# ThotDjehuty/polaroid

Hardware: AMD Instinct MI355X
Metric: Mrows/sec filter+groupby-agg on 1e9-row f64/i64; achieved HBM GB/s vs peak (higher is better)
Workload: dtype f64; 1 GPU; filter(close > 250).group_by(symbol).agg(open/high/low/close.sum()) 1e+09 rows per GPU, 100 groups (metric size; configs[1] = 1e8 rows); rows_per_gpu=1000000000, groups=100, global_batch=1000000000, columns=symbol:i64 open,high,low,close:f64, parallelism=single GPU

## Files before the change

### polaroid_amd/csrc/groupby.hip

```cpp
#include <hip/hip_runtime.h>

#include <algorithm>
#include <cmath>
#include <cstdio>
#include <cstdlib>
#include <cstring>
#include <mutex>
#include <numeric>
#include <string>
#include <tuple>
#include <vector>

#include "groupby_kernels.hpp"

namespace plgpu {

static int d2h_stage(int n, void* const* dst, const void* const* src, const size_t* bytes, hipStream_t s) {
    return plgpu_memcpy_d2h_many(n, dst, src, bytes, (void*)s);
}


#ifdef PLGPU_CHECKS
static std::vector<GbChecksTake>& gb_checks_takers() {
    static std::vector<GbChecksTake> v;
// ... 622 lines not shown
                }
                if ((x & 0x7fffffffffffffffull) != 0 && ex != 0x7FF && el < mn) mn = el;
            }
        }
    }
#pragma unroll
    for (int off = 32; off >= 1; off >>= 1) {
        const uint32_t o = __shfl_xor(mx, off, 64);
        mx = mx > o ? mx : o;
        const uint32_t q = __shfl_xor(mn, off, 64);
        mn = mn < q ? mn : q;
    }
    if ((threadIdx.x & 63) == 0) {
        red[0][threadIdx.x >> 6] = mx;
        red[1][threadIdx.x >> 6] = mn;
    }
    __syncthreads();
    if (threadIdx.x == 0) {
        for (int w = 1; w < kPlanThreads / 64; ++w) {
            mx = red[0][w] > mx ? red[0][w] : mx;
            mn = red[1][w] < mn ? red[1][w] : mn;
        }
        if (mx) atomicMax((unsigned long long*)&p.status[ST_MAXEX + a], (unsigned long long)mx);
        if (mn != 0x7FF) atomicMax((unsigned long long*)&p.status[ST_MINEX + a], (unsigned long long)(0x7FF - mn));
    }
}

static int32_t plan_bottom(uint64_t maxex) {
    int e = maxex == 0 ? 2046 : (int)maxex + kHeadroomBinades;
    if (e > 2046) e = 2046;
    return e - 1075 - (kSumWindowBits - 53);
}

__global__ void gb_init_table_kernel(uint64_t* gtab, int64_t words_per_field, int nfields, uint64_t min_init_mask) {
    for (int f = 0; f < nfields; ++f) {
        const uint64_t v = f == 0 ? kEmptyKey : (((min_init_mask >> f) & 1ull) ? ~0ull : 0ull);
        uint64_t* q = gtab + (int64_t)f * words_per_field;
        for (int64_t i = (int64_t)blockIdx.x * blockDim.x + threadIdx.x; i < words_per_field;
             i += (int64_t)gridDim.x * blockDim.x)
            q[i] = v;
    }
}


constexpr int kVarWords = 16;

__device__ __forceinline__ bool abs192(uint64_t& w0, uint64_t& w1, uint64_t& w2) {
    const bool neg = (int64_t)w2 < 0;
    if (neg) {
        w0 = ~w0; w1 = ~w1; w2 = ~w2;
        w0 += 1;
        const uint64_t c0 = w0 == 0;
        w1 += c0;
        w2 += (c0 && w1 == 0) ? 1 : 0;
    }
    return neg;
}

__device__ bool big_add_shifted(uint64_t (&acc)[kVarWords], const uint64_t* m, int k, int sh, bool negate) {
    int top = k - 1;
    while (top >= 0 && m[top] == 0) --top;
    if (top < 0) return true;
    const int bitlen = top * 64 + 64 - __clzll(m[top]);
    if (sh < 0 || bitlen + sh > kVarWords * 64 - 2) return false;
    const int ws = sh >> 6, bs = sh & 63;
    uint64_t carry = negate ? 1 : 0;
    for (int i = 0; i < kVarWords; ++i) {
// ... 786 lines not shown
            continue;
        }
        if (lp.n != 3 || lp.code[2].arg != PLGPU_F64) continue;
        int32_t op;
        switch (lp.code[2].op) {
        case D_ADD_F: op = DOP_ADD; break;
        case D_SUB_F: op = DOP_SUB; break;
        case D_MUL_F: op = DOP_MUL; break;
        case D_DIV_F: op = DOP_DIV; break;
        case D_DIV_FS: op = DOP_DIVS; break;
        default: continue;
        }
        const DevInstr &i0 = lp.code[0], &i1 = lp.code[1];
        auto f64col = [&](const DevInstr& i) { return i.op == D_COL && cols[i.arg].dtype == PLGPU_F64; };
        if (f64col(i0) && f64col(i1)) {
            di.kind = 2, di.ca = i0.arg, di.cb = i1.arg, di.dop = op;
        } else if (f64col(i0) && i1.op == D_LIT) {
            di.kind = 2, di.ca = i0.arg, di.dop = op | DOP_LIT, di.imm = i1.imm;
        } else if (i0.op == D_LIT && f64col(i1)) {
            di.kind = 2, di.ca = i1.arg, di.dop = op | DOP_LIT | DOP_SWAP, di.imm = i0.imm;
        }
    }
    return PLGPU_OK;
}

struct GbRun {
    Plan pl;
    DevProgram dp;
    int pred = 0;
    hipStream_t s = nullptr;
    DevBuf<uint64_t> status;
    int32_t* bottoms = nullptr;
    DevBuf<uint64_t> gtab;
    uint64_t st[ST_WORDS];
    int32_t hb[kMaxAcc];
    int gbits = 10;
    int attempts = 0;
    float ms = 0.f;
    int32_t key_dtype = PLGPU_I64;
    bool maintain = false;
    bool want_first = false;
    int world = 1;
    uint32_t wide = 0;
    int wide_exmin[kMaxAcc] = {0};
    int wide_exmax[kMaxAcc] = {0};
    DevBuf<int64_t> wide_digits[kMaxAcc];
    DevBuf<double> wide_sum[kMaxAcc];
    int64_t est_groups = -1;
    bool wide_round = true;
    std::string plan_ckey;
    bool kp_fallback = false;
    bool kp_bad = false;
    bool part = false;
    int pbits = 0;
    int part_lbits = 0;
    int part_blocks = 1;
    int part_levels = 0;
    int rbits = 0;
    bool compact_ok = false;
    bool compact_now = false;
    DevBuf<uint32_t> region_cnt;
    DevBuf<uint64_t> rtab;
    bool has_null_key = false;
    int64_t null_key = 0;
    DevBuf<uint64_t> pbuf;
    DevBuf<uint64_t> prange;
// ... 800 lines not shown
                                  160 * 1024);
        attr_set = true;
    }
    DevProgram none;
    std::memset(&none, 0, sizeof none);
    gb_kernel<0, true, true><<<(1 << R.pbits) * R.part_blocks, kGbThreads, lds, R.s>>>(q, none);
    return hipGetLastError();
}

static int gb_alloc_table(GbRun& R) {
    GbParams& p = R.pl.p;
    R.gtab.reset();
    R.rtab.reset();
    p.rtab = nullptr;
    p.rcap = 0;
    p.region_cnt = nullptr;
    p.gbits = R.gbits;
    p.rbits = R.rbits;
    if (R.compact_now) {
        p.rcap = int64_t(1) << (R.pbits + R.part_lbits);
        int rc = R.rtab.alloc((size_t)p.rcap * p.nfields * 8, R.s);
        if (rc) return rc;
        p.rtab = R.rtab;
        p.region_cnt = R.region_cnt;
        p.gbits = std::max(16, R.pbits + 2);
        p.rbits = 0;
    }
    p.gcap = int64_t(1) << p.gbits;
    const size_t wpf = (size_t)(p.gcap + 2);
    int rc = R.gtab.alloc(wpf * p.nfields * 8, R.s);
    if (rc) return rc;
    p.gtab = R.gtab;
    const int ig = (int)std::min<int64_t>((int64_t)(wpf + 255) / 256, 256 * 8);
    gb_init_table_kernel<<<ig, 256, 0, R.s>>>(R.gtab, (int64_t)wpf, p.nfields, p.min_init_mask);
    PLGPU_HIP(hipMemsetAsync(R.status, 0, 6 * 8, R.s));
    PLGPU_HIP(hipMemsetAsync(R.status + ST_MAXEX, 0, (ST_WORDS - ST_MAXEX) * 8, R.s));
    PLGPU_HIP(hipGetLastError());
    return PLGPU_OK;
}

static int gb_refit(GbRun& R, uint32_t flagged, int32_t* hint, bool* changed, uint32_t* wide) {
    GbParams& p = R.pl.p;
    *changed = false;
    *wide = 0;
    for (int a = 0; a < kMaxAcc; ++a) hint[a] = R.hb[a];
    if (!flagged) return PLGPU_OK;
    for (int a = 0; a < p.nacc; ++a)
        if ((flagged >> a) & 1u) gb_maxexp_kernel<<<std::max(1, num_cus() * 4), 256, 0, R.s>>>(p, a);
    PLGPU_HIP(hipGetLastError());
    if (int rs = d2h_status(R)) return rs;
    for (int a = 0; a < p.nacc; ++a) {
        if (!((flagged >> a) & 1u)) continue;
        const int tmax = std::max((int)R.st[ST_MAXEX + a], 1);
        const int tmin = std::max(0x7FF - (int)R.st[ST_MINEX + a], 1);
        if (tmax - tmin <= kSumWindowBits - 53) {
            hint[a] = tmax - 1075 - (kSumWindowBits - 53);
            *changed = *changed || hint[a] != R.hb[a];
        } else {
            *wide |= 1u << a;
            R.wide_exmin[a] = std::min(tmin, tmax);
            R.wide_exmax[a] = tmax;
        }
    }
    return PLGPU_OK;
}

static int gb_wide(GbRun& R, bool round = true) {
// ... 1743 lines not shown
```

### polaroid_amd/csrc/groupby_kernels.hpp

```cpp
#pragma once
#include <hip/hip_runtime.h>

#include <algorithm>
#include <cmath>
#include <cstdio>
#include <cstdlib>
#include <cstring>
#include <mutex>
#include <numeric>
#include <optional>
#include <string>
#include <tuple>
#include <vector>

#include "plgpu_internal.hpp"
#include "scan.hpp"
#include "tuplehash.hpp"

namespace plgpu {

constexpr int kGbThreads = 512;
constexpr int kMaxAcc = 6;
constexpr int kMaxFields = 48;
constexpr int kLdsProbe = 16;
constexpr int kGlobalProbe = 4096;
constexpr int kLimb2Margin = 4;
constexpr int slim_vwords(int nacc) { return (1 + 3 * nacc) | 1; }
constexpr int slim_words(int nacc) { return 1 + slim_vwords(nacc); }
constexpr int kMinTilesPerWg = 160;
constexpr int kGridRounds = 8;
constexpr int kHeadroomBinades = 8;
constexpr int64_t kMaxRowsPerWg = int64_t(1) << 22;
constexpr int kPlanSamples = 65536;
constexpr int kPlanSetSlots = 4096;
constexpr int kPlanSetWord = 32;

enum : int32_t { A_FSUM = 1, A_FSUMCAST = 2, A_ISUM = 4, A_CNT = 8, A_MIN = 16, A_MAX = 32, A_FLAGS = 64 };
enum : uint8_t { FOP_NONE = 0, FOP_ADD = 1, FOP_MIN = 2, FOP_MAX = 3, FOP_OR = 4, FOP_ADD192 = 5, FOP_SKIP = 6 };
enum : uint32_t { FL_NAN = 1, FL_PINF = 2, FL_NINF = 4 };
enum : int {
    ST_NEWKEYS = 0,
    ST_GLOBAL_ROWS = 1,
    ST_TABLE_FULL = 2,
    ST_SELECTED = 3,
    ST_SPECIAL = 4,
    ST_GROUPS_OUT = 5,
    ST_DISTINCT = 6,
    ST_SAMPLED = 7,
    ST_MAXEX = 8,
    ST_FXFLAGS = 16,
    ST_SHIFT_OVF = 14,
    ST_MINEX = 17,
    ST_RUNS = 23,
    ST_LOCAL = 24,
    ST_VAR_OUT = 25,
    ST_KPACK = 26,
    ST_WORDS = 27
};

enum : int32_t { DOP_NONE = 0, DOP_ADD = 1, DOP_SUB = 2, DOP_MUL = 3, DOP_DIV = 4, DOP_DIVS = 5, DOP_SQHI = 6,
                 DOP_SQLO = 7, DOP_OPMASK = 7, DOP_SWAP = 8, DOP_LIT = 16 };

struct AccSpec {
    DevCol c;
    int32_t flags;
// ... 39 lines not shown
    int32_t _pad2;
    int32_t nacc;
    int32_t nfields;
    AccSpec acc[kMaxAcc];
    uint64_t desc[kMaxAcc];
    int32_t bottom[kMaxAcc];
    uint8_t fop[kMaxFields];
    int32_t pred_acc;
    int32_t f_len;
    int32_t f_first;
    int32_t f_last;
    int32_t lbits;
    uint64_t min_init_mask;
    int32_t lcap;
    int32_t gbits;
    int64_t gcap;
    uint64_t* gtab;
    const int32_t* bottoms;
    uint64_t* status;
    const uint64_t* part_range;
    const uint32_t* part_rows;
    const uint8_t* part_nulls;
    int32_t part_blocks;
    int32_t tiles_per_wg;
    int32_t rbits;
    int32_t vwords;
    KeyPack kp;
    uint32_t* region_cnt;
    uint64_t* rtab;
    int64_t rcap;
    int32_t wave_report;
    int32_t has_null_key;
    int64_t null_key;
};

enum : uint32_t {
    CK_LDS_SLOT = 1,
    CK_GLOBAL_SLOT = 2,
    CK_FAST_SLOT = 4,
    CK_FIRST_ROW = 8,
    CK_MERGE_SLOT = 16,
    CK_REP_ROW = 32,
    CK_VERIFY_SLOT = 64,
    CK_PART_POS = 128,
    CK_KEY_ROW = 256,
    CK_PERM = 512,
    CK_FIELD = 1024,
    CK_REGION = 2048
};
#ifdef PLGPU_CHECKS
using GbChecksTake = uint32_t (*)();
void gb_checks_register(GbChecksTake f);
static __device__ unsigned int g_gb_checks;
static __device__ unsigned long long g_gb_sink;
static uint32_t gb_checks_take_local() {
    uint32_t v = 0, z = 0;
    (void)hipMemcpyFromSymbol(&v, HIP_SYMBOL(g_gb_checks), sizeof v);
    (void)hipMemcpyToSymbol(HIP_SYMBOL(g_gb_checks), &z, sizeof z);
    return v;
}
static const bool g_gb_checks_registered = (gb_checks_register(&gb_checks_take_local), true);
__device__ __forceinline__ bool gb_ok(bool c, uint32_t bit) {
    if (!c) atomicOr(&g_gb_checks, bit);
    return c;
}
__device__ __forceinline__ unsigned long long* gb_sink() { return &g_gb_sink; }
// ... 610 lines not shown
                if (s >= 0) {
                    apply_row<true, kMaxAcc>(p, lds, L, s, row, rv, vm[0], dd, bot, nacc, d);
                } else {
                    ++d.nglobal;
                    global_row<kMaxAcc>(p, key[0], s != kGlobalNull, row, rv, vm[0], dd, bot, nacc, d);
                }
            }
            slot[0] = slot[1]; slot[1] = slot[2]; slot[2] = slot[3];
            vm[0] = vm[1]; vm[1] = vm[2]; vm[2] = vm[3];
            key[0] = key[1]; key[1] = key[2]; key[2] = key[3];
#pragma unroll
            for (int a = 0; a < kMaxAcc; ++a) {
                v[a][0] = v[a][1];
                v[a][1] = v[a][2];
                v[a][2] = v[a][3];
            }
        }
    }
    flush_and_report<USE_LDS>(p, lds, L, d);
}

constexpr int kKpFast = 2;
template <int NACC, int ROWS, bool DERIV = false, int PACK = 0, bool NUL = false>
struct FastTile {
    uint64_t key[ROWS];
    uint64_t kr[PACK ? kKpFast : 1][ROWS];
    uint64_t v[NACC > 0 ? NACC : 1][ROWS];
    uint64_t w[DERIV && NACC > 0 ? NACC : 1][ROWS];
    uint64_t pv[ROWS];
    uint32_t nv[NUL ? (ROWS + 1) / 2 : 1];
    uint32_t nr[NUL ? (ROWS + 1) / 2 : 1][NUL ? (NACC > 0 ? NACC : 1) + 2 : 1];
};

__device__ __forceinline__ int64_t fast_row(int64_t t, int T, int rows, int j) {
    return t * (int64_t)T * rows + (int64_t)(j >> 1) * 2 * T + 2 * threadIdx.x + (j & 1);
}

typedef unsigned long long u64x2_t __attribute__((ext_vector_type(2)));

template <bool NT>
__device__ __forceinline__ u64x2_t ld16(const uint64_t* p) {
    if (NT) return __builtin_nontemporal_load(reinterpret_cast<const u64x2_t*>(p));
    return *reinterpret_cast<const u64x2_t*>(p);
}

template <int NACC, int PRED, int ROWS, bool DERIV, int PACK, bool NUL = false>
__device__ __forceinline__ void fast_load_tail(const GbParams& p, int64_t t,
                                               FastTile<NACC, ROWS, DERIV, PACK, NUL>& x) {
    const int T = blockDim.x;
    const uint64_t* kp = (const uint64_t*)p.key.values + p.key.offset;
#pragma unroll
    for (int j = 0; j < ROWS; ++j) {
        const int64_t r = fast_row(t, T, ROWS, j);
        const bool in = r < p.n;
        if (PACK == 2) {
            const int64_t* o = (const int64_t*)p.kp.c[0].values + p.kp.c[0].offset;
            x.kr[0][j] = in ? (uint64_t)o[r] : 0ull;
            x.kr[1][j] = in ? (uint64_t)o[r + 1] : 0ull;
        } else if (PACK == 1) {
#pragma unroll
            for (int i = 0; i < kKpFast; ++i) x.kr[i][j] = in && i < p.kp.n ? dev_load(p.kp.c[i], r) : 0ull;
        } else {
            x.key[j] = in && p.key.values ? kp[r] : 0ull;
        }
#pragma unroll
        for (int c = 0; c < NACC; ++c) {
            if (!DERIV || p.acc[c].v_from < 0)
                x.v[c][j] = in ? ((const uint64_t*)p.acc[c].c.values + p.acc[c].c.offset)[r] : 0ull;
            if (DERIV && p.acc[c].dop != DOP_NONE && !(p.acc[c].dop & DOP_LIT) && p.acc[c].w_from < 0)
                x.w[c][j] = in ? ((const uint64_t*)p.acc[c].c2.values + p.acc[c].c2.offset)[r] : 0ull;
        }
        if (PRED == 1 && p.pred_acc < 0) x.pv[j] = in ? ((const uint64_t*)p.pred_col.values + p.pred_col.offset)[r] : 0ull;
    }
}

typedef unsigned int u32x2_t __attribute__((ext_vector_type(2)));

template <int NACC, int PRED, int ROWS, bool NT, bool DERIV, int PACK, bool NUL = false>
__device__ __forceinline__ void fast_load(const GbParams& p, int64_t t, FastTile<NACC, ROWS, DERIV, PACK, NUL>& x,
                                          int64_t rbase = 0, int64_t rmax = -1) {
    const int T = blockDim.x;
    const uint64_t* kp = (const uint64_t*)p.key.values + p.key.offset;
#pragma unroll
    for (int q = 0; q < ROWS / 2; ++q) {
        int64_t r = rbase + fast_row(t, T, ROWS, 2 * q);
        if (rmax >= 0) r = r < rmax ? r : rmax;
        if (PACK == 2) {
            const int64_t* o = (const int64_t*)p.kp.c[0].values + p.kp.c[0].offset + r;
            const u64x2_t a = ld16<NT>((const uint64_t*)o);
            const uint64_t e = NT ? __builtin_nontemporal_load((const uint64_t*)o + 2) : ((const uint64_t*)o)[2];
            x.kr[0][2 * q] = a.x;
            x.kr[0][2 * q + 1] = a.y;
            x.kr[1][2 * q] = a.y;
            x.kr[1][2 * q + 1] = e;
        } else if (PACK == 1) {
#pragma unroll
            for (int i = 0; i < kKpFast; ++i) {
                if (i >= p.kp.n) {
                    x.kr[i][2 * q] = x.kr[i][2 * q + 1] = 0;
                    continue;
                }
                const DevCol& kc = p.kp.c[i];
                if (kc.dtype == PLGPU_I64) {
                    const u64x2_t a = ld16<NT>((const uint64_t*)kc.values + kc.offset + r);
                    x.kr[i][2 * q] = a.x;
                    x.kr[i][2 * q + 1] = a.y;
                } else {
                    const u32x2_t* ap = reinterpret_cast<const u32x2_t*>((const uint32_t*)kc.values + kc.offset + r);
                    const u32x2_t a = NT ? __builtin_nontemporal_load(ap) : *ap;
                    x.kr[i][2 * q] = a.x;
                    x.kr[i][2 * q + 1] = a.y;
                }
            }
        } else if (p.key.values) {
            const u64x2_t a = ld16<NT>(kp + r);
            x.key[2 * q] = a.x;
            x.key[2 * q + 1] = a.y;
        } else {
// ... 11 lines not shown
                const uint64_t* wp = (const uint64_t*)p.acc[c].c2.values + p.acc[c].c2.offset;
                const u64x2_t w = ld16<NT>(wp + r);
                x.w[c][2 * q] = w.x;
                x.w[c][2 * q + 1] = w.y;
            }
        }
        if (PRED == 1 && p.pred_acc < 0) {
            const uint64_t* pp = (const uint64_t*)p.pred_col.values + p.pred_col.offset;
            const u64x2_t b = ld16<NT>(pp + r);
            x.pv[2 * q] = b.x;
            x.pv[2 * q + 1] = b.y;
        }
    }
}

__device__ __forceinline__ uint64_t pair_bit(const DevCol& c, int64_t r) {
    return ((uint64_t)(uintptr_t)c.validity & 3u) * 8u + (uint64_t)(c.offset + r);
}

__device__ __forceinline__ uint32_t pair_word(const DevCol& c, int64_t r) {
    if (!c.validity) return ~0u;
    const uint32_t* w = (const uint32_t*)((uintptr_t)c.validity & ~(uintptr_t)3);
    return __builtin_nontemporal_load(w + (pair_bit(c, r) >> 5));
}

__device__ __forceinline__ uint32_t pair_word_wave(const DevCol& c, int64_t rw) {
    if (!c.validity) return ~0u;
    const int lane = threadIdx.x & 63;
    const uint64_t b = (uint64_t)(c.offset + rw) + 2u * (uint32_t)lane;
    return __builtin_nontemporal_load((const uint32_t*)c.validity + (b >> 5));
}

template <int NACC, int PRED, int ROWS, bool PART, bool DERIV, int PACK, bool NUL>
__device__ __forceinline__ void fast_nulls(const GbParams& p, int64_t t, FastTile<NACC, ROWS, DERIV, PACK, NUL>& x,
                                           int64_t rbase, int64_t rmax, bool full) {
    if constexpr (NUL) {
        const int T = blockDim.x;
#pragma unroll
        for (int q = 0; q < ROWS / 2; ++q) {
            int64_t r = rbase + fast_row(t, T, ROWS, 2 * q);
            if (rmax >= 0) r = r < rmax ? r : rmax;
            if (PART) {
                x.nr[q][0] = p.part_nulls ? __builtin_nontemporal_load((const uint16_t*)(p.part_nulls + r)) : 0u;
            } else if (full && p.vwords) {
                const int64_t rw = r - 2 * (threadIdx.x & 63);
#pragma unroll
                for (int c = 0; c < NACC; ++c) x.nr[q][c] = pair_word_wave(p.acc[c].c, rw);
                x.nr[q][NACC] = pair_word_wave(p.key, rw);
                x.nr[q][NACC + 1] = PRED == 1 && p.pred_acc < 0 ? pair_word_wave(p.pred_col, rw) : ~0u;
            } else if (r < p.n) {
#pragma unroll
                for (int c = 0; c < NACC; ++c) x.nr[q][c] = pair_word(p.acc[c].c, r);
                x.nr[q][NACC] = pair_word(p.key, r);
                x.nr[q][NACC + 1] = PRED == 1 && p.pred_acc < 0 ? pair_word(p.pred_col, r) : ~0u;
            } else {
#pragma unroll
                for (int c = 0; c < NACC + 2; ++c) x.nr[q][c] = ~0u;
            }
        }
    }
}

template <int NACC, int PRED, int ROWS, bool PART, bool DERIV, int PACK, bool NUL>
__device__ __forceinline__ void fast_nulls_finish(const GbParams& p, int64_t t,
                                                  FastTile<NACC, ROWS, DERIV, PACK, NUL>& x, int64_t rbase,
                                                  int64_t rmax) {
    if constexpr (NUL) {
        const int T = blockDim.x;
#pragma unroll
        for (int q = 0; q < ROWS / 2; ++q) {
            if (PART) {
                x.nv[q] = x.nr[q][0];
                continue;
            }
            int64_t r = rbase + fast_row(t, T, ROWS, 2 * q);
            if (rmax >= 0) r = r < rmax ? r : rmax;
            auto bits = [&](const DevCol& c, uint32_t w) -> uint32_t {
                return ~(w >> ((uint32_t)pair_bit(c, r) & 31u)) & 3u;
            };
            uint32_t m = 0;
#pragma unroll
            for (int c = 0; c < NACC; ++c) {
                const uint32_t b = bits(p.acc[c].c, x.nr[q][c]);
                m |= ((b & 1u) << c) | ((b >> 1) << (8 + c));
            }
            const uint32_t bk = bits(p.key, x.nr[q][NACC]);
            m |= ((bk & 1u) << 6) | ((bk >> 1) << 14);
            if (PRED == 1) {
                const uint32_t bp = bits(p.pred_col, x.nr[q][NACC + 1]);
                m |= ((bp & 1u) << 7) | ((bp >> 1) << 15);
            }
            x.nv[q] = m;
        }
    }
}

template <int NACC, int ROWS, bool DERIV, int PACK, bool NUL = false>
__device__ __forceinline__ void fast_share(const int32_t (&vf)[NACC > 0 ? NACC : 1],
                                           const int32_t (&wf)[NACC > 0 ? NACC : 1],
                                           FastTile<NACC, ROWS, DERIV, PACK, NUL>& x) {
    if (!DERIV) return;
#pragma unroll
    for (int c = 0; c < NACC; ++c)
#pragma unroll
        for (int b = 0; b < NACC; ++b)
#pragma unroll
            for (int j = 0; j < ROWS; ++j) {
                if (b == vf[c]) x.v[c][j] = x.v[b][j];
// ... 36 lines not shown
    load_descs(p, dd0, bot0);
    int32_t dop0[NA], vf0[NA], wf0[NA];
    uint64_t dim0[NA];
#pragma unroll
    for (int a = 0; a < NA; ++a) {
        dop0[a] = DERIV && a < NACC ? p.acc[a].dop : DOP_NONE;
        dim0[a] = DERIV && a < NACC ? p.acc[a].dimm : 0ull;
        vf0[a] = DERIV && a < NACC ? p.acc[a].v_from : -1;
        wf0[a] = DERIV && a < NACC ? p.acc[a].w_from : -1;
    }
    __syncthreads();

    const int T = blockDim.x;
    int64_t ntiles = p.n_full / ((int64_t)T * ROWS);
    int64_t nall = ntiles + (p.n > p.n_full ? 1 : 0);
    int64_t t = blockIdx.x, tstep = gridDim.x;
    int64_t rbase = 0, rlo = 0, rhi = 0, rmax = -1;
    if (!PART && p.tiles_per_wg > 0) {
        t = (int64_t)blockIdx.x * p.tiles_per_wg;
        nall = std::min<int64_t>(nall, t + p.tiles_per_wg);
        tstep = 1;
    }
    if (PART) {
        const int q = blockIdx.x / p.part_blocks;
        rlo = (int64_t)p.part_range[q];
        rhi = (int64_t)p.part_range[q + 1];
        rbase = rlo & ~int64_t(1);
        rmax = p.n & ~int64_t(1);
        ntiles = (rhi - rbase + (int64_t)T * ROWS - 1) / ((int64_t)T * ROWS);
        nall = ntiles;
        t = blockIdx.x % p.part_blocks;
        tstep = p.part_blocks;
    }
    auto load_tile = [&](int64_t tt, FastTile<NL, ROWS, DERIV, PACK, NULLS>& x) {
        fast_nulls<NL, PRED, ROWS, PART, DERIV, PACK, NULLS>(p, tt, x, rbase, rmax, tt < ntiles);
        if (PART || tt < ntiles) fast_load<NL, PRED, ROWS, true, DERIV, PACK, NULLS>(p, tt, x, rbase, rmax);
        else fast_load_tail<NL, PRED, ROWS, DERIV, PACK, NULLS>(p, tt, x);
    };
    const int pbit = p.pred_acc >= 0 ? p.pred_acc : 7;
    uint64_t kpm[kKpFast], kpx[kKpFast], kpc[kKpFast];
    int32_t kpsh[kKpFast];
#pragma unroll
    for (int i = 0; i < kKpFast; ++i) {
        const bool on = PACK && i < p.kp.n;
        const int32_t dt = on ? p.kp.c[i].dtype : PLGPU_I64;
        kpm[i] = (dt == PLGPU_I32 || dt == PLGPU_U32) ? 0xFFFFFFFFull : ~0ull;
        kpx[i] = dt == PLGPU_I32 ? 0x80000000ull : 0ull;
        kpc[i] = kpx[i] + (on ? p.kp.base[i] : 0ull);
        kpsh[i] = on ? p.kp.shift[i] : 0;
    }
    const bool kpid = PACK == 1 && p.kp.n == 1 && p.kp.bits[0] >= 64 && p.kp.base[0] == 0 &&
                      p.kp.shift[0] == 0;
    constexpr uint32_t VM = (1u << NACC) - 1u;
    constexpr bool RACC = SUMONLY && LIMBS == 2 && RUNS;
    constexpr int KR = RACC ? (PART ? 4 : 1) : 1;
    int rs[KR];
    uint64_t rn[KR], rlo_[KR][NA], rhi_[KR][NA];
#pragma unroll
    for (int k = 0; k < KR; ++k) {
        rs[k] = -1;
        rn[k] = 0;
#pragma unroll
        for (int a = 0; a < NA; ++a) rlo_[k][a] = rhi_[k][a] = 0;
    }
    int rvict = 0;
    auto racc_flush = [&](int k) {
        if (rs[k] < 0) return;
        atomicAdd(fld(rs[k], 1), (unsigned long long)rn[k]);
#pragma unroll
        for (int a = 0; a < NACC; ++a) {
// ... 57 lines not shown
            const bool uns = (dsc >> 57) & 1;
            const uint64_t ab = x[a] & 0x7fffffffffffffffull;
            if (isf && ab >= 0x7ff0000000000000ull) {
                atomicOr(q + dfield(dsc, 48) * L, (unsigned long long)(ab > 0x7ff0000000000000ull ? FL_NAN
                                                                     : ((x[a] >> 63) ? FL_NINF : FL_PINF)));
            } else if (isf && (flags & A_FSUM)) {
                uint64_t l0, l1, l2;
                if (fx_limbs_fast<2>(x[a], bot0[a], l0, l1, l2)) {
                    gr0[a] += l0;
                    gr1[a] += l1;
                } else {
                    uint32_t ex = 0, fl = 0;
                    const bool ok = fx_limbs(x[a], bot0[a], l0, l1, l2, fl, ex);
                    d.fxbits |= fl << (2 * a);
                    if (ok) {
                        const int f = dfield(dsc, 8);
                        atomicAdd(q + f * L, (unsigned long long)l0);
                        atomicAdd(q + (f + 1) * L, (unsigned long long)l1);
                        atomicAdd(q + (f + 2) * L, (unsigned long long)l2);
                    }
                }
            } else if (!isf && (flags & A_ISUM)) {
                gr0[a] += x[a];
            }
            if (!(isf && ab > 0x7ff0000000000000ull)) {
                const uint64_t o = isf ? ord_f64(x[a]) : (uns ? x[a] : ord_i64(x[a]));
                gmin[a] = std::min(gmin[a], o);
                gmax[a] = std::max(gmax[a], o);
            }
        }
        return true;
    };
    FastTile<NL, ROWS, DERIV, PACK, NULLS> cur;
    if (t < nall) load_tile(t, cur);
    for (; t < nall; t += tstep) {
        if constexpr (!VAR) fast_share<NACC, ROWS, DERIV, PACK, NULLS>(vf0, wf0, cur);
        fast_nulls_finish<NL, PRED, ROWS, PART, DERIV, PACK, NULLS>(p, t, cur, rbase, rmax);
        bool kout[ROWS];
        constexpr bool kstr = PACK == 2;
        if (kstr) {
#pragma unroll
            for (int j = 0; j < ROWS; ++j) {
                kout[j] = false;
                cur.key[j] = kp_str_code(p.kp.c[0].data, p.kp.data_end, cur.kr[0][j], cur.kr[1][j] - cur.kr[0][j],
                                         kout[j]);
            }
        }
        if (PACK == 1 && kpid) {
#pragma unroll
            for (int j = 0; j < ROWS; ++j) {
                kout[j] = false;
                cur.key[j] = ((cur.kr[0][j] & kpm[0]) ^ kpx[0]) - kpx[0];
            }
        }
#pragma unroll
        for (int j = 0; j < ROWS; ++j) {
            if (!kstr) kout[j] = false;
        }
        if (PACK == 1 && !kpid) {
#pragma unroll
            for (int j = 0; j < ROWS; ++j) cur.key[j] = 0;
#pragma unroll
            for (int i = 0; i < kKpFast; ++i) {
                if (i >= p.kp.n) continue;
                const int md = p.kp.mode[i];
                if (md == 0) {
#pragma unroll
                    for (int j = 0; j < ROWS; ++j) {
                        const uint64_t f = cur.kr[i][j] - kpc[i];
                        kout[j] |= f > p.kp.span[i];
// ... 7 lines not shown
                        cur.key[j] |= (uint64_t)f << kpsh[i];
                    }
                } else {
#pragma unroll
                    for (int j = 0; j < ROWS; ++j) {
                        const uint64_t f = ((cur.kr[i][j] & kpm[i]) ^ kpx[i]) - kpc[i];
                        kout[j] |= f > p.kp.span[i];
                        cur.key[j] |= f << kpsh[i];
                    }
                }
            }
        }
        int slot[ROWS];
        uint64_t probe[ROWS];
        uint32_t h[ROWS];
        uint32_t nrw[ROWS];
#pragma unroll
        for (int j = 0; j < ROWS; ++j) {
            nrw[j] = NULLS ? (cur.nv[j >> 1] >> (8 * (j & 1))) & 0xFFu : 0u;
            bool sel = true;
            if (PRED == 1) {
                uint64_t x = cur.pv[j];
                if (TRIPLE) {
                    if (p.pred_acc >= 0) x = cur.v[0][j];
                } else {
#pragma unroll
                    for (int a = 0; a < NACC; ++a)
                        if (a == p.pred_acc) x = cur.v[a][j];
                }
                sel = simple_pred(prog.simple_isf, prog.simple_op, x, prog.simple_imm);
                if (NULLS) sel = sel && !((nrw[j] >> pbit) & 1u);
            }
            if (PART) {
                const int64_t r = rbase + fast_row(t, T, ROWS, j);
                sel = r >= rlo && r < rhi;
            } else if (t >= ntiles) {
                sel = sel && fast_row(t, T, ROWS, j) < p.n;
            }
            if (PACK && sel && kout[j]) d.kbad = 1u;
            const bool knull = (NULLS && ((nrw[j] >> 6) & 1u)) ||
                               (PART && p.has_null_key && cur.key[j] == (uint64_t)p.null_key);
            slot[j] = sel ? (knull ? p.lcap : (cur.key[j] == kEmptyKey ? p.lcap + 1 : kGlobalKey)) : kNotSelected;
            h[j] = hash_slot(cur.key[j], p.lbits);
            probe[j] = lds_load(&lds[h[j]]);
        }
#pragma unroll
        for (int j = 0; j < ROWS; ++j)
            if (slot[j] == kGlobalKey && probe[j] == cur.key[j]) slot[j] = (int)h[j];
        FastTile<NL, ROWS, DERIV, PACK, NULLS> nxt;
        const int64_t tn = t + tstep;
        if (tn < nall) load_tile(tn, nxt);
#pragma unroll 1
        for (int j = 0; j < ROWS; ++j) {
            const int64_t r = rbase + fast_row(t, T, ROWS, j);
            int s = slot[0];
            if (s != kNotSelected) {
                ++d.nsel;
                uint64_t rv[NA], dd[NA];
                int bot[NA];
#pragma unroll
                for (int a = 0; a < NA; ++a) {
                    if (TRIPLE) {
                        rv[a] = a == 0 ? cur.v[0][0] : derive(a == 1 ? DOP_SQHI : DOP_SQLO, cur.v[0][0], 0ull);
                    } else if (VAR == 2 || VAR == 3) {
                        rv[a] = a == VAR - 2 ? f64_bits(as_f64(cur.v[0][0]) * as_f64(cur.v[1][0])) : cur.v[a][0];
                    } else {
                        rv[a] = cur.v[a][0];
                        if (DERIV && dop0[a] != DOP_NONE)
                            rv[a] = derive(dop0[a], cur.v[a][0], (dop0[a] & DOP_LIT) ? dim0[a] : cur.w[a][0]);
                    }
                    dd[a] = dd0[a];
                    bot[a] = bot0[a];
                    if (NULLS && SUMONLY && ((nrw[0] >> a) & 1u)) rv[a] = 0ull;
                }
                const uint32_t vm = NULLS ? VM & ~nrw[0] : VM;
                if (s == kGlobalKey) s = lds_find(lds, p.lbits, p.lcap, cur.key[0]);
                if (s >= 0 && !gb_ok(s < L, CK_FAST_SLOT)) s = -1;
                bool held = false;
                if (RACC && s >= 0) {
                    uint64_t lo[NA], hi[NA];
                    bool ok = true;
#pragma unroll
                    for (int a = 0; a < NACC; ++a) {
                        uint64_t l0, l1, l2;
                        ok = fx_limbs_fast<LIMBS>(rv[a], bot[a], l0, l1, l2) && ok;
                        lo[a] = l0;
                        hi[a] = l1;
// ... 75 lines not shown
                                const bool ok = LIMBS == 3
                                                    ? fx_limbs<kSumWindowBits>(x, bot[a], l0, l1, l2, fl, ex)
                                                    : fx_limbs<kSumWindowBits - 40>(x, bot[a] + 40, l0, l1, l2, fl,
                                                                                    ex);
                                d.fxbits |= fl << (2 * a);
                                if (ok) {
                                    if (LIMBS == 3) atomicAdd(fld(s, 2 + 4 * a), (unsigned long long)l0);
                                    atomicAdd(fld(s, so_mid(a)), (unsigned long long)(LIMBS == 3 ? l1 : l0));
                                    atomicAdd(fld(s, so_top(a)), (unsigned long long)(LIMBS == 3 ? l2 : l1));
                                }
                            }
                        }
                    }
                } else if (s >= 0) {
                    if (!grun_take(s, r, rv)) apply_row<true, NA>(p, lds, L, s, r, rv, vm, dd, bot, NACC, d);
                } else {
                    ++d.nglobal;
                    global_row<NA>(p, cur.key[0], true, r, rv, vm, dd, bot, NACC, d);
                }
            }
#pragma unroll
            for (int i = 0; i + 1 < ROWS; ++i) {
                slot[i] = slot[i + 1];
                nrw[i] = nrw[i + 1];
                cur.key[i] = cur.key[i + 1];
#pragma unroll
                for (int a = 0; a < NL; ++a) {
                    cur.v[a][i] = cur.v[a][i + 1];
                    if (DERIV) cur.w[a][i] = cur.w[a][i + 1];
                }
            }
        }
        cur = nxt;
    }
    if (RACC) {
#pragma unroll
        for (int k = 0; k < KR; ++k) racc_flush(k);
    }
    if (SLIM) {
        __syncthreads();
        uint32_t* wsc = (uint32_t*)&lds[(size_t)L * slim_words(NACC)];
        auto store_slot = [&](int sl, uint64_t* tab, int64_t stride, int64_t t, uint64_t len) {
            tab[(int64_t)p.f_len * stride + t] = len;
#pragma unroll
            for (int a = 0; a < NACC; ++a) {
                const int f = p.acc[a].f_sum;
                uint64_t w0, w1, w2;
                limbs_to_192(0, (int64_t)*fld(sl, so_mid(a)), (int64_t)*fld(sl, so_top(a)), w0, w1, w2);
                tab[(int64_t)f * stride + t] = w0;
                tab[(int64_t)(f + 1) * stride + t] = w1;
                tab[(int64_t)(f + 2) * stride + t] = w2;
                tab[(int64_t)p.acc[a].f_flags * stride + t] = *fld(sl, so_flags(a));
            }
        };
        auto add_slot = [&](int sl, int64_t gs, uint64_t len) {
            atomicAdd((unsigned long long*)gfield(p, p.f_len, gs), (unsigned long long)len);
#pragma unroll
            for (int a = 0; a < NACC; ++a) {
                const int f = p.acc[a].f_sum;
                uint64_t w0, w1, w2;
                limbs_to_192(0, (int64_t)*fld(sl, so_mid(a)), (int64_t)*fld(sl, so_top(a)), w0, w1, w2);
                g_add192(gfield(p, f, gs), gfield(p, f + 1, gs), gfield(p, f + 2, gs), w0, w1, w2);
                const uint64_t fl = *fld(sl, so_flags(a));
                if (fl) atomicOr((unsigned long long*)gfield(p, p.acc[a].f_flags, gs), (unsigned long long)fl);
            }
        };
// ... 113 lines not shown
}

inline bool same_dev_col(const DevCol& x, const DevCol& y) {
    return x.values == y.values && x.offset == y.offset && x.dtype == y.dtype && x.validity == y.validity;
}

inline void pair_normalize(GbParams& q, int pi, bool pred) {
    AccSpec& pa = q.acc[pi];
    if (!same_dev_col(pa.c2, q.acc[1 - pi].c)) std::swap(pa.c, pa.c2);
    if (pred) {
        q.pred_acc = -1;
        for (int a = 0; a < 2 && q.pred_acc < 0; ++a)
            if (same_dev_col(q.acc[a].c, q.pred_col)) q.pred_acc = a;
    }
}

template <int NACC, int PRED, bool SUMONLY, int LIMBS = 3, bool RUNS = false, bool DERIV = false, int VAR = 0,
          int PACK = 0, int ROWS = 2, bool NULLS = false>
hipError_t launch_fast_rows(const Plan& pl, const DevProgram& dp, hipStream_t s) {
    const void* kern =
        (const void*)gb_fast_kernel<NACC, PRED, SUMONLY, ROWS, LIMBS, RUNS, false, DERIV, VAR, PACK, NULLS>;
    static bool attr_set = false;
    if (!attr_set) {
        (void)hipFuncSetAttribute(kern, hipFuncAttributeMaxDynamicSharedMemorySize, 160 * 1024);
        attr_set = true;
    }
    const size_t lds =
        (SUMONLY && LIMBS == 2) ? (size_t)slim_words(NACC) * (pl.p.lcap + 2) * 8 + kWgScratch : pl.lds_bytes;
    GbParams q = pl.p;
    q.tiles_per_wg = 0;
    q.wave_report = options().wave_report;
    if (VAR == 2 || VAR == 3) pair_normalize(q, VAR - 2, PRED == 1);
    if (ROWS != 2) q.n_full = (pl.p.n / ((int64_t)kGbThreads * ROWS)) * kGbThreads * ROWS;
    const int64_t need = (q.n_full + kMaxRowsPerWg - 1) / kMaxRowsPerWg;
    const int64_t useful = q.n_full / ((int64_t)kGbThreads * ROWS);
    const int64_t resident = (int64_t)num_cus() * resident_per_cu(kern, kGbThreads, lds);
    const int64_t rounds = options().grid_rounds > 0
                               ? options().grid_rounds
                               : std::min<int64_t>(kGridRounds, std::max<int64_t>(1, useful / (resident * kMinTilesPerWg)));
    int64_t g = resident * rounds;
    if (g < need) g = need;
    if (g > useful) g = std::max<int64_t>(1, useful);
    const int grid = (int)g;
    pl.launched_grid = grid;
    pl.launched_runs = RUNS;
    pl.launched_var = VAR == 1 || VAR == 4;
    static_assert(VAR < 8 && PACK < 4 && LIMBS < 4 && NACC < 8 && PRED < 2 && ROWS < 16, "fused_variant's fields");
    pl.launched_variant = VAR | PACK << 3 | (NULLS ? 1 : 0) << 5 | (RUNS ? 1 : 0) << 6 | (DERIV ? 1 : 0) << 7 |
                          LIMBS << 8 | NACC << 10 | PRED << 13 | (SUMONLY ? 1 : 0) << 14 | 1 << 15 | ROWS << 16 |
                          (NULLS && q.vwords ? 1 : 0) << 20;
    if (pl.local) {
        const int64_t tile = (int64_t)kGbThreads * ROWS;
        const int64_t nall = q.n_full / tile + (pl.p.n > q.n_full ? 1 : 0);
        q.tiles_per_wg = (int32_t)((nall + grid - 1) / grid);
    }
    KtScope kt(q.wave_report ? "gb_fast_wave_report_kernel" : "gb_fast_kernel", s);
    gb_fast_kernel<NACC, PRED, SUMONLY, ROWS, LIMBS, RUNS, false, DERIV, VAR, PACK, NULLS>
        <<<grid, kGbThreads, lds, s>>>(q, dp);
    return hipGetLastError();
}

inline bool var_x_nonneg(const Plan& pl, const DevProgram& dp, int a = 0) {
    if (!dp.simple || !dp.simple_isf || pl.p.pred_acc != a || dp.simple_op < 0 || dp.simple_op > 5) return false;
    if (pl.p.acc[a].dop != DOP_NONE || pl.p.acc[a].c.dtype != PLGPU_F64) return false;
    const uint32_t accept = (0x643152u >> (4 * dp.simple_op)) & 0xFu;
    if (accept & 1u) return false;
    double c;
    std::memcpy(&c, &dp.simple_imm, 8);
    return c >= 0.0;
}

template <int NACC>
hipError_t launch_fast_nulls(const Plan& pl, const DevProgram& dp, int pred, hipStream_t s) {
    if constexpr (NACC > 0) {
        if (pl.sum_only && pl.limbs == 2 && pred == 1 && options().sum_pos && var_x_nonneg(pl, dp, NACC - 1))
            return launch_fast_rows<NACC, 1, true, 2, false, false, 5, 0, 2, true>(pl, dp, s);
        if (pl.sum_only && pl.limbs == 2)
            return pred == 0 ? launch_fast_rows<NACC, 0, true, 2, false, false, 0, 0, 2, true>(pl, dp, s)
                             : launch_fast_rows<NACC, 1, true, 2, false, false, 0, 0, 2, true>(pl, dp, s);
    }
    return pred == 0 ? launch_fast_rows<NACC, 0, false, 3, false, false, 0, 0, 2, true>(pl, dp, s)
                     : launch_fast_rows<NACC, 1, false, 3, false, false, 0, 0, 2, true>(pl, dp, s);
}

template <int NACC, int PRED, bool SUMONLY, bool DERIV, int PACK = 0>
hipError_t launch_fast(const Plan& pl, const DevProgram& dp, hipStream_t s) {
    if (SUMONLY && pl.limbs == 2 && pl.runs)
        return launch_fast_rows<NACC, PRED, SUMONLY, 2, true, DERIV, false, PACK>(pl, dp, s);
    if constexpr (NACC == 4 && PRED == 1 && SUMONLY && !DERIV) {
// ... 168 lines not shown
```

### polaroid_amd/csrc/plgpu_internal.hpp

```cpp
#pragma once

#include <hip/hip_runtime.h>
#include <stdint.h>

#include <cstring>

#include <string>
#include <vector>

#include "../../include/polaroid_gpu.h"

#define PLGPU_API extern "C" __attribute__((visibility("default")))

namespace plgpu {

void set_error(const std::string& msg);
int fail(int code, const std::string& msg);
int hip_fail(hipError_t e, const char* what);

#define PLGPU_HIP(expr)                                   \
    do {                                                  \
        hipError_t _e = (expr);                           \
        if (_e != hipSuccess) return plgpu::hip_fail(_e, #expr); \
    } while (0)

hipStream_t as_stream(void* s);

struct Options {
    int debug = 0;
    int no_pack = 0;
    int mk_collide = 0;
    int runs = -1;
    int local = -1;
    int ktime = 0;
    int fuse_keys = 1;
    int plan_cache = 1;
    int grid_rounds = 0;
    int gb_path = -1;
    int part_bits = -1;
    int part_levels = -1;
    int part_direct = 1;
    int part_lds_kb = 0;
    int part_compact = 1;
    int rl_stream = 0;
    int rl_grid = 0;
    int filt_pipe = 1;
    int part_threads = 0;
    int rl_div = 1;
    int rl_full = 1;
    int rl_mean_hot = 1;
    int rl_var_hot = 1;
    int rl_var128 = 1;
    int alloc_skew = 0;
    int alloc_contig = 0;
    int srt_w4 = 0;
    int srt_up_tiles = 1;
    int part_rows4 = 0;
    int wave_report = 0;
    int part_null_sentinel = 1;
    int filt_fused = 0;
    int var_pos = 1;
    int sum_pos = 1;
    int gb_pair = 1;
    int join_radix = 1;
    int join_radix_keys = 0;
    int join_radix_load = 0;
    int join_radix_batch = 0;
    int over_presorted = 1;
    int asof_path = 0;
};
// ... 704 lines not shown
```

### polaroid_amd/csrc/runtime.cpp

```cpp
#include <hip/hip_runtime.h>

#include <cstdio>
#include <cstdlib>
#include <algorithm>
#include <cmath>
#include <cstdint>
#include <cstring>
#include <map>
#include <mutex>
#include <string>
#include <unordered_map>
#include <vector>

#include "plgpu_internal.hpp"

namespace plgpu {

static thread_local std::string g_last_error;

void set_error(const std::string& msg) { g_last_error = msg; }

int fail(int code, const std::string& msg) {
    g_last_error = msg;
    return code;
// ... 25 lines not shown
    {"plan_cache", "PLGPU_PLAN_CACHE", &Options::plan_cache},
    {"gb_path", "PLGPU_GB_PATH", &Options::gb_path},
    {"part_bits", "PLGPU_PART_BITS", &Options::part_bits},
    {"part_levels", "PLGPU_PART_LEVELS", &Options::part_levels},
    {"part_direct", "PLGPU_PART_DIRECT", &Options::part_direct},
    {"part_compact", "PLGPU_PART_COMPACT", &Options::part_compact},
    {"rl_var128", "PLGPU_RL_VAR128", &Options::rl_var128},
    {"rl_var_hot", "PLGPU_RL_VAR_HOT", &Options::rl_var_hot},
    {"rl_mean_hot", "PLGPU_RL_MEAN_HOT", &Options::rl_mean_hot},
    {"over_presorted", "PLGPU_OVER_PRESORTED", &Options::over_presorted},
    {"alloc_skew", "PLGPU_ALLOC_SKEW", &Options::alloc_skew},
    {"alloc_contig", "PLGPU_ALLOC_CONTIG", &Options::alloc_contig},
    {"srt_w4", "PLGPU_SRT_W4", &Options::srt_w4},
    {"srt_up_tiles", "PLGPU_SRT_UP_TILES", &Options::srt_up_tiles},
    {"part_rows4", "PLGPU_PART_ROWS4", &Options::part_rows4},
    {"wave_report", "PLGPU_WAVE_REPORT", &Options::wave_report},
    {"part_null_sentinel", "PLGPU_PART_NULL_SENTINEL", &Options::part_null_sentinel},
    {"part_lds_kb", "PLGPU_PART_LDS_KB", &Options::part_lds_kb},
    {"rl_stream", "PLGPU_RL_STREAM", &Options::rl_stream},
    {"rl_grid", "PLGPU_RL_GRID", &Options::rl_grid},
    {"filt_pipe", "PLGPU_FILT_PIPE", &Options::filt_pipe},
    {"rl_div", "PLGPU_RL_DIV", &Options::rl_div},
    {"part_threads", "PLGPU_PART_THREADS", &Options::part_threads},
    {"gb_pair", "PLGPU_GB_PAIR", &Options::gb_pair},
    {"rl_full", "PLGPU_RL_FULL", &Options::rl_full},
    {"filt_fused", "PLGPU_FILT_FUSED", &Options::filt_fused},
    {"var_pos", "PLGPU_VAR_POS", &Options::var_pos},
    {"sum_pos", "PLGPU_SUM_POS", &Options::sum_pos},
    {"join_radix", "PLGPU_JOIN_RADIX", &Options::join_radix},
    {"join_radix_keys", "PLGPU_JOIN_RADIX_KEYS", &Options::join_radix_keys},
    {"join_radix_load", "PLGPU_JOIN_RADIX_LOAD", &Options::join_radix_load},
    {"join_radix_batch", "PLGPU_JOIN_RADIX_BATCH", &Options::join_radix_batch},
    {"asof_path", "PLGPU_ASOF_PATH", &Options::asof_path},
};
const OptField* opt_field(const char* name) {
    for (const OptField& f : kOptFields)
        if (!strcmp(name, f.name)) return &f;
    return nullptr;
}
}

static Options read_env_options() {
    Options o;
    for (const OptField& f : kOptFields) {
        const char* e = getenv(f.env);
        if (e) o.*(f.f) = atoi(e);
    }
    return o;
}

Options& options() {
    static Options o = read_env_options();
    return o;
}

namespace {
struct KtPending {
    const char* name;
    hipEvent_t a, b;
};
struct KtSum {
    std::string name;
    double ms = 0.0;
    int64_t count = 0;
};
std::mutex g_kt_mu;
// ... 801 lines not shown
```

Measured before the change: 151,500 Mrows/s.

## Add per-wave dynamic tile claiming with segmented atomic counters in fast groupby

Replaces the static grid-stride tile assignment in the fast groupby kernel with per-wavefront dynamic work claiming. 64 segmented atomic counters hand out chunks of 64-row-wide tiles, and a wave that drains its segment steals from the segment with the most work left. The grid is sized to the resident capacity instead of several rounds. The aim is to remove tail imbalance between workgroups and waves on a bandwidth-bound scan, at the cost of atomics, a wave-wide steal search, and narrower per-wave tiles that could hurt coalescing.

Result: faster. 156,100 Mrows/s (median of 6 runs) (+3.1%).

```diff
diff --git a/polaroid_amd/csrc/groupby.hip b/polaroid_amd/csrc/groupby.hip
--- a/polaroid_amd/csrc/groupby.hip
+++ b/polaroid_amd/csrc/groupby.hip
@@ -678,7 +678,10 @@
     return e - 1075 - (kSumWindowBits - 53);
 }
 
-__global__ void gb_init_table_kernel(uint64_t* gtab, int64_t words_per_field, int nfields, uint64_t min_init_mask) {
+__global__ void gb_init_table_kernel(uint64_t* gtab, int64_t words_per_field, int nfields, uint64_t min_init_mask,
+                                     uint32_t* claim) {
+    if (blockIdx.x == 0 && claim)
+        for (int i = threadIdx.x; i < kClaimSegs * kClaimStride; i += blockDim.x) claim[i] = 0u;
     for (int f = 0; f < nfields; ++f) {
         const uint64_t v = f == 0 ? kEmptyKey : (((min_init_mask >> f) & 1ull) ? ~0ull : 0ull);
         uint64_t* q = gtab + (int64_t)f * words_per_field;
@@ -1531,6 +1534,7 @@
     DevBuf<uint64_t> status;
     int32_t* bottoms = nullptr;
     DevBuf<uint64_t> gtab;
+    DevBuf<uint32_t> claim;
     uint64_t st[ST_WORDS];
     int32_t hb[kMaxAcc];
     int gbits = 10;
@@ -2397,7 +2401,9 @@
     if (rc) return rc;
     p.gtab = R.gtab;
     const int ig = (int)std::min<int64_t>((int64_t)(wpf + 255) / 256, 256 * 8);
-    gb_init_table_kernel<<<ig, 256, 0, R.s>>>(R.gtab, (int64_t)wpf, p.nfields, p.min_init_mask);
+    if (R.claim == nullptr && (rc = R.claim.alloc((size_t)kClaimSegs * kClaimStride * 4, R.s))) return rc;
+    p.claim = R.claim;
+    gb_init_table_kernel<<<ig, 256, 0, R.s>>>(R.gtab, (int64_t)wpf, p.nfields, p.min_init_mask, p.claim);
     PLGPU_HIP(hipMemsetAsync(R.status, 0, 6 * 8, R.s));
     PLGPU_HIP(hipMemsetAsync(R.status + ST_MAXEX, 0, (ST_WORDS - ST_MAXEX) * 8, R.s));
     PLGPU_HIP(hipGetLastError());
diff --git a/polaroid_amd/csrc/groupby_kernels.hpp b/polaroid_amd/csrc/groupby_kernels.hpp
--- a/polaroid_amd/csrc/groupby_kernels.hpp
+++ b/polaroid_amd/csrc/groupby_kernels.hpp
@@ -31,6 +31,9 @@
 constexpr int kGridRounds = 8;
 constexpr int kHeadroomBinades = 8;
 constexpr int64_t kMaxRowsPerWg = int64_t(1) << 22;
+constexpr int kClaimSegs = 64;
+constexpr int kClaimChunk = 8;
+constexpr int kClaimStride = 32;
 constexpr int kPlanSamples = 65536;
 constexpr int kPlanSetSlots = 4096;
 constexpr int kPlanSetWord = 32;
@@ -136,6 +139,13 @@
     int32_t wave_report;
     int32_t has_null_key;
     int64_t null_key;
+    uint32_t* claim;
+    int32_t claim_segs;
+    int32_t claim_chunk;
+    int32_t claim_cap;
+    int32_t _pad3;
+    int64_t claim_seg_units;
+    int64_t claim_units;
 };
 
 enum : uint32_t {
@@ -812,8 +822,8 @@
     uint32_t nr[NUL ? (ROWS + 1) / 2 : 1][NUL ? (NACC > 0 ? NACC : 1) + 2 : 1];
 };
 
-__device__ __forceinline__ int64_t fast_row(int64_t t, int T, int rows, int j) {
-    return t * (int64_t)T * rows + (int64_t)(j >> 1) * 2 * T + 2 * threadIdx.x + (j & 1);
+__device__ __forceinline__ int64_t fast_row(int64_t base, int W, int i, int j) {
+    return base + (int64_t)(j >> 1) * 2 * W + 2 * i + (j & 1);
 }
 
 typedef unsigned long long u64x2_t __attribute__((ext_vector_type(2)));
@@ -825,13 +835,12 @@
 }
 
 template <int NACC, int PRED, int ROWS, bool DERIV, int PACK, bool NUL = false>
-__device__ __forceinline__ void fast_load_tail(const GbParams& p, int64_t t,
+__device__ __forceinline__ void fast_load_tail(const GbParams& p, int64_t base, int W, int i,
                                                FastTile<NACC, ROWS, DERIV, PACK, NUL>& x) {
-    const int T = blockDim.x;
     const uint64_t* kp = (const uint64_t*)p.key.values + p.key.offset;
 #pragma unroll
     for (int j = 0; j < ROWS; ++j) {
-        const int64_t r = fast_row(t, T, ROWS, j);
+        const int64_t r = fast_row(base, W, i, j);
         const bool in = r < p.n;
         if (PACK == 2) {
             const int64_t* o = (const int64_t*)p.kp.c[0].values + p.kp.c[0].offset;
@@ -857,13 +866,12 @@
 typedef unsigned int u32x2_t __attribute__((ext_vector_type(2)));
 
 template <int NACC, int PRED, int ROWS, bool NT, bool DERIV, int PACK, bool NUL = false>
-__device__ __forceinline__ void fast_load(const GbParams& p, int64_t t, FastTile<NACC, ROWS, DERIV, PACK, NUL>& x,
-                                          int64_t rbase = 0, int64_t rmax = -1) {
-    const int T = blockDim.x;
+__device__ __forceinline__ void fast_load(const GbParams& p, int64_t base, int W, int i,
+                                          FastTile<NACC, ROWS, DERIV, PACK, NUL>& x, int64_t rmax = -1) {
     const uint64_t* kp = (const uint64_t*)p.key.values + p.key.offset;
 #pragma unroll
     for (int q = 0; q < ROWS / 2; ++q) {
-        int64_t r = rbase + fast_row(t, T, ROWS, 2 * q);
+        int64_t r = fast_row(base, W, i, 2 * q);
         if (rmax >= 0) r = r < rmax ? r : rmax;
         if (PACK == 2) {
             const int64_t* o = (const int64_t*)p.kp.c[0].values + p.kp.c[0].offset + r;
@@ -941,13 +949,12 @@
 }
 
 template <int NACC, int PRED, int ROWS, bool PART, bool DERIV, int PACK, bool NUL>
-__device__ __forceinline__ void fast_nulls(const GbParams& p, int64_t t, FastTile<NACC, ROWS, DERIV, PACK, NUL>& x,
-                                           int64_t rbase, int64_t rmax, bool full) {
+__device__ __forceinline__ void fast_nulls(const GbParams& p, int64_t base, int W, int i,
+                                           FastTile<NACC, ROWS, DERIV, PACK, NUL>& x, int64_t rmax, bool full) {
     if constexpr (NUL) {
-        const int T = blockDim.x;
 #pragma unroll
         for (int q = 0; q < ROWS / 2; ++q) {
-            int64_t r = rbase + fast_row(t, T, ROWS, 2 * q);
+            int64_t r = fast_row(base, W, i, 2 * q);
             if (rmax >= 0) r = r < rmax ? r : rmax;
             if (PART) {
                 x.nr[q][0] = p.part_nulls ? __builtin_nontemporal_load((const uint16_t*)(p.part_nulls + r)) : 0u;
@@ -971,18 +978,16 @@
 }
 
 template <int NACC, int PRED, int ROWS, bool PART, bool DERIV, int PACK, bool NUL>
-__device__ __forceinline__ void fast_nulls_finish(const GbParams& p, int64_t t,
-                                                  FastTile<NACC, ROWS, DERIV, PACK, NUL>& x, int64_t rbase,
-                                                  int64_t rmax) {
+__device__ __forceinline__ void fast_nulls_finish(const GbParams& p, int64_t base, int W, int i,
+                                                  FastTile<NACC, ROWS, DERIV, PACK, NUL>& x, int64_t rmax) {
     if constexpr (NUL) {
-        const int T = blockDim.x;
 #pragma unroll
         for (int q = 0; q < ROWS / 2; ++q) {
             if (PART) {
                 x.nv[q] = x.nr[q][0];
                 continue;
             }
-            int64_t r = rbase + fast_row(t, T, ROWS, 2 * q);
+            int64_t r = fast_row(base, W, i, 2 * q);
             if (rmax >= 0) r = r < rmax ? r : rmax;
             auto bits = [&](const DevCol& c, uint32_t w) -> uint32_t {
                 return ~(w >> ((uint32_t)pair_bit(c, r) & 31u)) & 3u;
@@ -1085,10 +1090,68 @@
         t = blockIdx.x % p.part_blocks;
         tstep = p.part_blocks;
     }
+    const bool dyn = !PART && p.claim != nullptr;
+    const int W = dyn ? 64 : T;
+    const int wi = dyn ? (int)(threadIdx.x & 63) : (int)threadIdx.x;
+    int64_t uend = 0;
+    int32_t seg = 0, ntaken = 0;
+    uint32_t pend = 0;
+    bool has_pend = false;
+    if (dyn) {
+        ntiles = p.n_full / (64 * ROWS);
+        nall = p.claim_units;
+        seg = (int32_t)(blockIdx.x % (uint32_t)p.claim_segs);
+    }
+    auto seg_len = [&](int64_t s_) -> int64_t {
+        const int64_t l = p.claim_units - s_ * p.claim_seg_units;
+        return l < 0 ? 0 : (l < p.claim_seg_units ? l : p.claim_seg_units);
+    };
+    auto claim_issue = [&]() {
+        has_pend = ntaken + p.claim_chunk <= p.claim_cap;
+        if (has_pend && (threadIdx.x & 63) == 0)
+            pend = __hip_atomic_fetch_add(p.claim + seg * kClaimStride, (uint32_t)p.claim_chunk, __ATOMIC_RELAXED,
+                                          __HIP_MEMORY_SCOPE_AGENT);
+    };
+    auto claim_take = [&](int64_t& tn) -> bool {
+        while (has_pend) {
+            const int64_t v = (int64_t)(uint32_t)__builtin_amdgcn_readfirstlane((int)pend);
+            const int64_t len = seg_len(seg);
+            if (v < len) {
+                tn = seg * p.claim_seg_units + v;
+                uend = seg * p.claim_seg_units + (v + p.claim_chunk < len ? v + p.claim_chunk : len);
+                ntaken += p.claim_chunk;
+                has_pend = false;
+                return true;
+            }
+            const int ln = (int)(threadIdx.x & 63);
+            uint64_t left = 0;
+            if (ln < p.claim_segs) {
+                const int64_t c = (int64_t)__hip_atomic_load(p.claim + ln * kClaimStride, __ATOMIC_RELAXED,
+                                                             __HIP_MEMORY_SCOPE_AGENT);
+                const int64_t l = seg_len(ln);
+                left = l > c ? (uint64_t)(l - c) : 0ull;
+            }
+            unsigned long long best = (unsigned long long)(left << 6 | (uint64_t)ln);
+#pragma unroll
+            for (int off = 32; off > 0; off >>= 1) {
+                const unsigned long long o = __shfl_xor(best, off);
+                best = o > best ? o : best;
+            }
+            const uint32_t blo = (uint32_t)__builtin_amdgcn_readfirstlane((int)(uint32_t)best);
+            const uint32_t bhi = (uint32_t)__builtin_amdgcn_readfirstlane((int)(uint32_t)(best >> 32));
+            if ((((uint64_t)bhi << 32 | blo) >> 6) == 0) break;
+            seg = (int32_t)(blo & 63u);
+            claim_issue();
+        }
+        has_pend = false;
+        return false;
+    };
+    auto tile_base = [&](int64_t tt) -> int64_t { return rbase + tt * (int64_t)W * ROWS; };
     auto load_tile = [&](int64_t tt, FastTile<NL, ROWS, DERIV, PACK, NULLS>& x) {
-        fast_nulls<NL, PRED, ROWS, PART, DERIV, PACK, NULLS>(p, tt, x, rbase, rmax, tt < ntiles);
-        if (PART || tt < ntiles) fast_load<NL, PRED, ROWS, true, DERIV, PACK, NULLS>(p, tt, x, rbase, rmax);
-        else fast_load_tail<NL, PRED, ROWS, DERIV, PACK, NULLS>(p, tt, x);
+        const int64_t tb = tile_base(tt);
+        fast_nulls<NL, PRED, ROWS, PART, DERIV, PACK, NULLS>(p, tb, W, wi, x, rmax, tt < ntiles);
+        if (PART || tt < ntiles) fast_load<NL, PRED, ROWS, true, DERIV, PACK, NULLS>(p, tb, W, wi, x, rmax);
+        else fast_load_tail<NL, PRED, ROWS, DERIV, PACK, NULLS>(p, tb, W, wi, x);
     };
     const int pbit = p.pred_acc >= 0 ? p.pred_acc : 7;
     uint64_t kpm[kKpFast], kpx[kKpFast], kpc[kKpFast];
@@ -1212,10 +1275,16 @@
         return true;
     };
     FastTile<NL, ROWS, DERIV, PACK, NULLS> cur;
-    if (t < nall) load_tile(t, cur);
-    for (; t < nall; t += tstep) {
+    bool have = t < nall;
+    if (dyn) {
+        claim_issue();
+        have = claim_take(t);
+        if (have && t + 1 == uend) claim_issue();
+    }
+    if (have) load_tile(t, cur);
+    while (have) {
         if constexpr (!VAR) fast_share<NACC, ROWS, DERIV, PACK, NULLS>(vf0, wf0, cur);
-        fast_nulls_finish<NL, PRED, ROWS, PART, DERIV, PACK, NULLS>(p, t, cur, rbase, rmax);
+        fast_nulls_finish<NL, PRED, ROWS, PART, DERIV, PACK, NULLS>(p, tile_base(t), W, wi, cur, rmax);
         bool kout[ROWS];
         constexpr bool kstr = PACK == 2;
         if (kstr) {
@@ -1289,10 +1358,10 @@
                 if (NULLS) sel = sel && !((nrw[j] >> pbit) & 1u);
             }
             if (PART) {
-                const int64_t r = rbase + fast_row(t, T, ROWS, j);
+                const int64_t r = fast_row(tile_base(t), W, wi, j);
                 sel = r >= rlo && r < rhi;
             } else if (t >= ntiles) {
-                sel = sel && fast_row(t, T, ROWS, j) < p.n;
+                sel = sel && fast_row(tile_base(t), W, wi, j) < p.n;
             }
             if (PACK && sel && kout[j]) d.kbad = 1u;
             const bool knull = (NULLS && ((nrw[j] >> 6) & 1u)) ||
@@ -1305,11 +1374,17 @@
         for (int j = 0; j < ROWS; ++j)
             if (slot[j] == kGlobalKey && probe[j] == cur.key[j]) slot[j] = (int)h[j];
         FastTile<NL, ROWS, DERIV, PACK, NULLS> nxt;
-        const int64_t tn = t + tstep;
-        if (tn < nall) load_tile(tn, nxt);
+        int64_t tn = t + tstep;
+        bool hn = tn < nall;
+        if (dyn) {
+            tn = t + 1;
+            hn = tn < uend || claim_take(tn);
+            if (hn && tn + 1 == uend) claim_issue();
+        }
+        if (hn) load_tile(tn, nxt);
 #pragma unroll 1
         for (int j = 0; j < ROWS; ++j) {
-            const int64_t r = rbase + fast_row(t, T, ROWS, j);
+            const int64_t r = fast_row(tile_base(t), W, wi, j);
             int s = slot[0];
             if (s != kNotSelected) {
                 ++d.nsel;
@@ -1451,6 +1526,8 @@
             }
         }
         cur = nxt;
+        t = tn;
+        have = hn;
     }
     if (RACC) {
 #pragma unroll
@@ -1630,15 +1707,39 @@
     q.wave_report = options().wave_report;
     if (VAR == 2 || VAR == 3) pair_normalize(q, VAR - 2, PRED == 1);
     if (ROWS != 2) q.n_full = (pl.p.n / ((int64_t)kGbThreads * ROWS)) * kGbThreads * ROWS;
-    const int64_t need = (q.n_full + kMaxRowsPerWg - 1) / kMaxRowsPerWg;
     const int64_t useful = q.n_full / ((int64_t)kGbThreads * ROWS);
     const int64_t resident = (int64_t)num_cus() * resident_per_cu(kern, kGbThreads, lds);
-    const int64_t rounds = options().grid_rounds > 0
-                               ? options().grid_rounds
-                               : std::min<int64_t>(kGridRounds, std::max<int64_t>(1, useful / (resident * kMinTilesPerWg)));
-    int64_t g = resident * rounds;
-    if (g < need) g = need;
-    if (g > useful) g = std::max<int64_t>(1, useful);
+    const bool claimable = !pl.local && options().grid_rounds == 0;
+    const bool claimed = claimable && options().gb_claim != 0 && q.claim != nullptr;
+    int64_t g;
+    if (claimed) {
+        constexpr int64_t unit = 64 * ROWS, waves = kGbThreads / 64;
+        const int64_t cap_rows =
+            options().claim_cap_rows > 0 ? std::min<int64_t>(options().claim_cap_rows, kMaxRowsPerWg) : kMaxRowsPerWg;
+        int64_t cap = std::max<int64_t>(1, cap_rows / (waves * unit));
+        const int64_t units = q.n_full / unit + (pl.p.n - q.n_full + unit - 1) / unit;
+        const int64_t chunk = std::min<int64_t>(
+            cap, std::max<int64_t>(1, std::min<int64_t>(kClaimChunk, units / (resident * waves * 4))));
+        cap -= cap % chunk;
+        q.claim_segs = kClaimSegs;
+        q.claim_chunk = (int32_t)chunk;
+        q.claim_cap = (int32_t)cap;
+        q.claim_seg_units = ((units + kClaimSegs - 1) / kClaimSegs + chunk - 1) / chunk * chunk;
+        q.claim_units = units;
+        const int64_t need = ((units + chunk - 1) / chunk * chunk + waves * cap - 1) / (waves * cap);
+        g = std::min<int64_t>(resident, std::max<int64_t>(1, useful));
+        if (g < need) g = need;
+    } else {
+        q.claim = nullptr;
+        const int64_t need = (q.n_full + kMaxRowsPerWg - 1) / kMaxRowsPerWg;
+        const int64_t rounds =
+            options().grid_rounds > 0
+                ? options().grid_rounds
+                : std::min<int64_t>(kGridRounds, std::max<int64_t>(1, useful / (resident * kMinTilesPerWg)));
+        g = resident * rounds;
+        if (g < need) g = need;
+        if (g > useful) g = std::max<int64_t>(1, useful);
+    }
     const int grid = (int)g;
     pl.launched_grid = grid;
     pl.launched_runs = RUNS;
@@ -1652,7 +1753,8 @@
         const int64_t nall = q.n_full / tile + (pl.p.n > q.n_full ? 1 : 0);
         q.tiles_per_wg = (int32_t)((nall + grid - 1) / grid);
     }
-    KtScope kt(q.wave_report ? "gb_fast_wave_report_kernel" : "gb_fast_kernel", s);
+    KtScope kt(q.wave_report ? "gb_fast_wave_report_kernel"
+                             : (claimable && !claimed ? "gb_fast_static_kernel" : "gb_fast_kernel"), s);
     gb_fast_kernel<NACC, PRED, SUMONLY, ROWS, LIMBS, RUNS, false, DERIV, VAR, PACK, NULLS>
         <<<grid, kGbThreads, lds, s>>>(q, dp);
     return hipGetLastError();
diff --git a/polaroid_amd/csrc/plgpu_internal.hpp b/polaroid_amd/csrc/plgpu_internal.hpp
--- a/polaroid_amd/csrc/plgpu_internal.hpp
+++ b/polaroid_amd/csrc/plgpu_internal.hpp
@@ -36,6 +36,8 @@
     int fuse_keys = 1;
     int plan_cache = 1;
     int grid_rounds = 0;
+    int gb_claim = 1;
+    int claim_cap_rows = 0;
     int gb_path = -1;
     int part_bits = -1;
     int part_levels = -1;
diff --git a/polaroid_amd/csrc/runtime.cpp b/polaroid_amd/csrc/runtime.cpp
--- a/polaroid_amd/csrc/runtime.cpp
+++ b/polaroid_amd/csrc/runtime.cpp
@@ -81,6 +81,8 @@
     {"join_radix_load", "PLGPU_JOIN_RADIX_LOAD", &Options::join_radix_load},
     {"join_radix_batch", "PLGPU_JOIN_RADIX_BATCH", &Options::join_radix_batch},
     {"asof_path", "PLGPU_ASOF_PATH", &Options::asof_path},
+    {"gb_claim", "PLGPU_GB_CLAIM", &Options::gb_claim},
+    {"claim_cap_rows", "PLGPU_CLAIM_CAP_ROWS", &Options::claim_cap_rows},
 };
 const OptField* opt_field(const char* name) {
     for (const OptField& f : kOptFields)
```
